# jontio/JAERO

Hardware: AMD Instinct MI355X
Metric: Msamples/s of real 48 kHz PCM through the 10.5 kbps OQPSK demodulator hot path (higher is better)
Workload: dtype f64; 1 GPU; 65536-channel-per-GPU synthetic 48 kHz 10.5 kbps OQPSK continuous (BASELINE configs[2] shape, scaled to 65536 channels per GPU = one wavefront of 64 channels per SIMD), 4096-sample writes, coarse 2^14 FFT every 4096 samples, AFC off, EbNo meters on, Eb/N0 10.0 dB, per-channel carrier (8000 +- 100 Hz), bits, noise, symbol phase; 42 untimed pre-roll steps (the last 14 resident and back to back with ; channels_per_gpu=65536, total_channels=65536, chunk=4096, ebno_meters=True, preroll_steps=42, timing_phases=32, hbm_bytes_per_resident_channel=2263808, resident_channels_max=136593, ranks=1, control_plane=none (single rank), sustain_steps=14

## Files before the change

### jaero_amd/csrc/k_coarse6.h

```cpp
#pragma once
#include "k_coarse2.h"

#ifndef C4_TABN
#define C4_TABN 3584
#endif
__device__ __forceinline__ void c6_bar() { asm volatile("s_waitcnt lgkmcnt(0)\n\ts_barrier" ::: "memory"); }
#define C6_FENCE __builtin_amdgcn_sched_barrier(0)
__device__ __forceinline__ double2 c6_sq(const double2 a)
{
#pragma clang fp contract(fast)
    return make_double2(a.x * a.x - a.y * a.y, 2.0 * (a.x * a.y));
}

#ifndef C6_TRACE
#define C6_TRACE(i)
#endif

template <int CTRL, int ROWMASK>
__device__ __forceinline__ void c6_argmax_step(double &bv, int &bi)
{
    const int lo = __builtin_amdgcn_update_dpp(__double2loint(bv), __double2loint(bv), CTRL, ROWMASK, 0xf, false);
    const int hi = __builtin_amdgcn_update_dpp(__double2hiint(bv), __double2hiint(bv), CTRL, ROWMASK, 0xf, false);
    const int oi = __builtin_amdgcn_update_dpp(bi, bi, CTRL, ROWMASK, 0xf, false);
    const double ov = __hiloint2double(hi, lo);
    const bool take = (oi >= 0) & ((bi < 0) | (ov > bv) | ((ov == bv) & (oi < bi)));
    bv = take ? ov : bv;
    bi = take ? oi : bi;
}
__device__ __forceinline__ void c6_wave_argmax(double &bv, int &bi)
{
    c6_argmax_step<0xB1, 0xf>(bv, bi);
    c6_argmax_step<0x4E, 0xf>(bv, bi);
    c6_argmax_step<0x141, 0xf>(bv, bi);
    c6_argmax_step<0x140, 0xf>(bv, bi);
    c6_argmax_step<0x142, 0xa>(bv, bi);
    c6_argmax_step<0x143, 0xc>(bv, bi);
    bv = __hiloint2double(__builtin_amdgcn_readlane(__double2hiint(bv), 63), __builtin_amdgcn_readlane(__double2loint(bv), 63));
    bi = __builtin_amdgcn_readlane(bi, 63);
}

#define C6_XCH 16448

__device__ __forceinline__ constexpr int c6_k(int s) { return s < 16 ? 2 * s : 2 * (s - 16) + 1; }

__device__ __forceinline__ void c6_fft32(CV<32> &x)
{
#pragma clang fp contract(fast)
#pragma unroll
    for (int j = 0; j < 16; j++)
    {
        const double ar = x.r[j], ai = x.i[j], br = x.r[j + 16], bi = x.i[j + 16];
        x.r[j] = ar + br; x.i[j] = ai + bi;
        double dr = ar - br, di = ai - bi;
        cmul_w64(dr, di, 2 * j);
        x.r[j + 16] = dr; x.i[j + 16] = di;
    }
    C6_FENCE;
#pragma unroll
    for (int h = 0; h < 2; h++)
    {
        CV<16> in, out;
#pragma unroll
        for (int j = 0; j < 16; j++) { in.r[j] = x.r[16 * h + j]; in.i[j] = x.i[16 * h + j]; }
        regfft<16>(in, out);
#pragma unroll
        for (int j = 0; j < 16; j++) { x.r[16 * h + j] = out.r[j]; x.i[16 * h + j] = out.i[j]; }
        C6_FENCE;
    }
}

__device__ __forceinline__ void c6_twiddle32(CV<32> &x, const double2 p1)
{
#pragma clang fp contract(fast)
    auto app = [&](int slot, const double2 w) __attribute__((always_inline)) {
        const double r = x.r[slot] * w.x - x.i[slot] * w.y, i = x.r[slot] * w.y + x.i[slot] * w.x;
        x.r[slot] = r; x.i[slot] = i;
    };
    const double2 p2 = c6_sq(p1);
    double2 e = p2;
    app(16, p1);
#pragma unroll
    for (int j = 1; j < 16; j++)
    {
        app(j, e);
        app(16 + j, cmul2(e, p1));
        if (j < 15) e = cmul2(e, p2);
    }
}

__device__ __forceinline__ void wg_fft14_e32(CV<32> &d, double *xch, const double2 *__restrict__ tw, int t)
{
#pragma clang fp contract(fast)
    const double2 st1 = tw[t], st2 = tw[32 * (t & 15)];
    const int k1u = t >> 4, n3 = t & 15, odd = k1u & 1;
    const int e1w0 = t, e1w1 = (t + 16) & 511;
    const int e1r = k1u * 512 + odd * 16 + n3;
    const int e1rw = e1r + 496 - 512 * odd;
    const int e2w = k1u + n3 * 513;
    const int e2r = t;

    c6_fft32(d);
    c6_twiddle32(d, st1);
    C6_FENCE;
    c6_bar();
#pragma unroll
    for (int s = 0; s < 32; s++) xch[c6_k(s) * 512 + ((c6_k(s) & 1) ? e1w1 : e1w0)] = d.r[s];
    c6_bar();
#pragma unroll
    for (int m = 0; m < 32; m++) d.r[m] = xch[(m < 31 ? e1r + 16 * m : e1rw)];
    c6_bar();
#pragma unroll
    for (int s = 0; s < 32; s++) xch[c6_k(s) * 512 + ((c6_k(s) & 1) ? e1w1 : e1w0)] = d.i[s];
    c6_bar();
#pragma unroll
    for (int m = 0; m < 32; m++) d.i[m] = xch[(m < 31 ? e1r + 16 * m : e1rw)];
    C6_FENCE;
    c6_fft32(d);
    c6_twiddle32(d, st2);
    C6_FENCE;
    c6_bar();
#pragma unroll
    for (int s = 0; s < 32; s++) xch[e2w + (c6_k(s) & 15) * 32 + (c6_k(s) >> 4) * 8208] = d.r[s];
    c6_bar();
#pragma unroll
    for (int m = 0; m < 32; m++) d.r[m] = xch[e2r + (m & 15) * 513 + (m >> 4) * 8208];
    c6_bar();
#pragma unroll
    for (int s = 0; s < 32; s++) xch[e2w + (c6_k(s) & 15) * 32 + (c6_k(s) >> 4) * 8208] = d.i[s];
    c6_bar();
#pragma unroll
    for (int m = 0; m < 32; m++) d.i[m] = xch[e2r + (m & 15) * 513 + (m >> 4) * 8208];
    C6_FENCE;
    {
        CV<16> in, o0, o1;
#pragma unroll
        for (int j = 0; j < 16; j++) { in.r[j] = d.r[j]; in.i[j] = d.i[j]; }
        regfft<16>(in, o0);
        C6_FENCE;
#pragma unroll
        for (int j = 0; j < 16; j++) { in.r[j] = d.r[16 + j]; in.i[j] = d.i[16 + j]; }
        regfft<16>(in, o1);
#pragma unroll
        for (int k3 = 0; k3 < 16; k3++) { d.r[2 * k3] = o0.r[k3]; d.i[2 * k3] = o0.i[k3]; d.r[2 * k3 + 1] = o1.r[k3]; d.i[2 * k3 + 1] = o1.i[k3]; }
    }
}


#define C6_XCH13 8208
__device__ __forceinline__ void wg_fft13_e32(CV<32> &d, double *xch, const double2 *__restrict__ tw, int t)
{
#pragma clang fp contract(fast)
    const double2 st1 = tw[t], st2 = tw[32 * (t & 15)];
    const int k1a = t >> 4, n3 = t & 15;
    const int e1r = k1a * 256 + n3;
    const int e2w = k1a + 513 * n3;
    c6_fft32(d);
    c6_twiddle32(d, st1);
    C6_FENCE;
    c6_bar();
#pragma unroll
    for (int s = 0; s < 32; s++) (xch + c6_k(s) * 256)[t] = d.r[s];
    c6_bar();
#pragma unroll
    for (int m = 0; m < 32; m++) d.r[m] = (xch + (m >> 4) * 4096 + (m & 15) * 16)[e1r];
    c6_bar();
#pragma unroll
    for (int s = 0; s < 32; s++) (xch + c6_k(s) * 256)[t] = d.i[s];
    c6_bar();
#pragma unroll
    for (int m = 0; m < 32; m++) d.i[m] = (xch + (m >> 4) * 4096 + (m & 15) * 16)[e1r];
    C6_FENCE;
#pragma unroll
    for (int g2 = 0; g2 < 2; g2++)
    {
        CV<16> in, out;
#pragma unroll
        for (int j = 0; j < 16; j++) { in.r[j] = d.r[16 * g2 + j]; in.i[j] = d.i[16 * g2 + j]; }
        regfft<16>(in, out);
        c4_twiddle16(out, st2);
#pragma unroll
        for (int j = 0; j < 16; j++) { d.r[16 * g2 + j] = out.r[j]; d.i[16 * g2 + j] = out.i[j]; }
        C6_FENCE;
    }
    c6_bar();
#pragma unroll
    for (int s = 0; s < 32; s++) (xch + (s >> 4) * 16 + (s & 15) * 32)[e2w] = d.r[s];
    c6_bar();
#pragma unroll
    for (int m = 0; m < 32; m++) d.r[m] = (xch + (m >> 4) * 256 + (m & 15) * 513)[t];
    c6_bar();
#pragma unroll
    for (int s = 0; s < 32; s++) (xch + (s >> 4) * 16 + (s & 15) * 32)[e2w] = d.i[s];
    c6_bar();
#pragma unroll
    for (int m = 0; m < 32; m++) d.i[m] = (xch + (m >> 4) * 256 + (m & 15) * 513)[t];
    C6_FENCE;
    {
        CV<16> in, o0, o1;
#pragma unroll
        for (int j = 0; j < 16; j++) { in.r[j] = d.r[j]; in.i[j] = d.i[j]; }
        regfft<16>(in, o0);
        C6_FENCE;
#pragma unroll
        for (int j = 0; j < 16; j++) { in.r[j] = d.r[16 + j]; in.i[j] = d.i[16 + j]; }
        regfft<16>(in, o1);
#pragma unroll
        for (int k3 = 0; k3 < 16; k3++) { d.r[2 * k3] = o0.r[k3]; d.i[2 * k3] = o0.i[k3]; d.r[2 * k3 + 1] = o1.r[k3]; d.i[2 * k3 + 1] = o1.i[k3]; }
    }
}

template <int LOG2N>
__device__ __forceinline__ void c6_fft(CV<32> &d, double *xch, const double2 *__restrict__ tw, int t)
{
    int tt = t;
    asm volatile("" : "+v"(tt));
    if constexpr (LOG2N == 14) wg_fft14_e32(d, xch, tw, tt);
    else wg_fft13_e32(d, xch, tw, tt);
}

__device__ __noinline__ void c6_build_window(double *wt, int startbin, int t, int nthreads)
{
    for (int i = t; i <= startbin + 1; i += nthreads)
    {
        const double c = cos(M_PI_2 * ((double)i) / ((double)startbin));
        wt[i] = (i == 0) ? 1.0 : ((i <= startbin) ? c * c : 0.0);
    }
}

template <bool W8400, int LOG2N = 14>
__device__ __forceinline__ void coarse6_body(const JGeom g, const JPtrs p, const int *__restrict__ chan_list, int nlist, const double2 *__restrict__ tw)
{
    constexpr int N = 1 << LOG2N;
    constexpr int E = 32;
    constexpr int NT = N / E;
    constexpr int XCH = LOG2N == 14 ? C6_XCH : C6_XCH13;
    extern __shared__ __attribute__((aligned(16))) double xch[];
    __shared__ double red_val[NT / 64];
    __shared__ int red_idx[NT / 64];
    const int t0 = threadIdx.x;
    const int nchp = g.nchp;
    int tab_startbin = -1;

    CV<E> d;
    int ch_next = ((int)blockIdx.x < nlist) ? (chan_list ? jd_sload(chan_list + blockIdx.x) : (int)blockIdx.x) : 0;
    int bp_next = jd_sload(p.I + (size_t)I_BB_PTR * nchp + ch_next);
    for (int li = blockIdx.x; li < nlist; li += gridDim.x)
    {
        int t = t0;
        asm volatile("" : "+v"(t));
        const int ch = ch_next, bb_ptr = bp_next;
        const double2 *__restrict__ ring = p.bbring + (size_t)ch * N;
        const int ln = li + (int)gridDim.x;
        const bool has_next = ln < nlist;
        if (has_next)
        {
            ch_next = chan_list ? jd_sload(chan_list + ln) : ln;
            bp_next = jd_sload(p.I + (size_t)I_BB_PTR * nchp + ch_next);
        }
        const double lockingbw = jd_sload(p.S + (size_t)S_LOCKINGBW * nchp + ch);
        double fs_l = g.Fs;
        asm volatile("" : "+s"(fs_l));
        int startbin, expectedpeakbin;
        {
            const double hzperbin = fs_l * (1.0 / ((double)N));
            startbin = __builtin_amdgcn_readfirstlane((int)fmax(round(lockingbw / hzperbin), 1.0));
            expectedpeakbin = __builtin_amdgcn_readfirstlane((int)round(g.fb / (2.0 * hzperbin)));
        }
        const int stopbin = N - startbin;
        double *__restrict__ y = p.y + (size_t)ch * N;

        if (li == (int)blockIdx.x)
        {
#pragma unroll
            for (int s = 0; s < E; s++)
            {
                const double2 v = ring[(bb_ptr + s * NT + t) & (N - 1)];
                d.r[s] = v.x; d.i[s] = v.y;
            }
        }
        C6_TRACE(0);
        c6_fft<LOG2N>(d, xch, tw, t);
        C6_TRACE(1);
        if constexpr (W8400)
        {
            const bool persistent = startbin < C4_TABN - 1;
            double *wt = persistent ? xch + XCH : xch;
            if (!persistent || startbin != tab_startbin)
            {
                c6_bar();
                c6_build_window(wt, startbin, t, NT);
                c6_bar();
                if (persistent) tab_startbin = startbin;
            }
#pragma unroll
            for (int s0 = 0; s0 < E; s0 += 8)
            {
#pragma unroll
                for (int s = s0; s < s0 + 8; s++)
                {
                    const int k = s * NT + t;
                    const int i = (k <= N / 2) ? k : N - k;
                    const double w = wt[i <= startbin ? i : startbin + 1];
                    const double re = d.r[s] * w, im = d.i[s] * w;
                    d.r[s] = im; d.i[s] = re;
                }
                C6_FENCE;
            }
            if (!persistent) c6_bar();
        }
        else
        {
#pragma unroll
            for (int s = 0; s < E; s++)
            {
                const int k = s * NT + t;
                const bool z = (k >= startbin) && (k <= stopbin);
                const double re = z ? 0.0 : d.r[s], im = z ? 0.0 : d.i[s];
                d.r[s] = im; d.i[s] = re;
            }
        }
        c6_fft<LOG2N>(d, xch, tw, t);
        C6_TRACE(2);
#pragma unroll
        for (int s = 0; s < E; s++)
        {
            const double re = d.i[s], im = d.r[s];
            d.r[s] = re * re - im * im;
            d.i[s] = re * im + im * re;
        }
        c6_fft<LOG2N>(d, xch, tw, t);
        C6_TRACE(3);
        c6_bar();
        CoarseSlotState cst;
        {
            double yv[E];
#pragma unroll
            for (int s = 0; s < E; s++) d.r[s] = d.r[s] * d.r[s] + d.i[s] * d.i[s];
            C6_FENCE;
#pragma unroll
            for (int s = 0; s < E; s++) yv[s] = __builtin_nontemporal_load((y + ((s * NT) ^ (N / 2))) + t);
            C6_FENCE;
            cst = coarse_slot_load_v(g, p, ch);
            int bpn = bp_next, chn = ch_next, tp = t;
            asm volatile("" : "+v"(bpn), "+v"(chn), "+v"(tp));
            typedef double c6_v2 __attribute__((ext_vector_type(2)));
            const c6_v2 *__restrict__ ringn = (const c6_v2 *)(p.bbring + (size_t)chn * N);
            const int toffp = bpn + tp;
#pragma unroll
            for (int s = 0; s < E; s++)
            {
                const int ib = (s * NT) ^ (N / 2);
                const double yn = yv[s] * 0.9 + 0.5 * jd_log10(fmax(d.r[s], 1.0));
                __builtin_nontemporal_store(yn, (y + ib) + t);
                (xch + ib)[t] = yn;
                {
                    const c6_v2 v = __builtin_nontemporal_load(ringn + ((toffp + s * NT) & (N - 1)));
                    d.r[s] = v.x; d.i[s] = v.y;
                }
                if ((s & 3) == 3) C6_FENCE;
            }
            C6_TRACE(4);
            c6_bar();
            C6_TRACE(5);
        }
        C6_TRACE(6);
        double fs_e = g.Fs;
        asm volatile("" : "+s"(fs_e));
        const double hzperbin = fs_e * (1.0 / ((double)N));
        const int i0 = __builtin_amdgcn_readfirstlane((int)round((-lockingbw / hzperbin) + ((double)(N / 2))));
        const int i1 = __builtin_amdgcn_readfirstlane((int)round((lockingbw / hzperbin) + ((double)(N / 2))));
        double best = 0;
        int besti = -1;
        const bool fold_inside = (i0 - expectedpeakbin - 1 >= 0) && (i1 + expectedpeakbin < N) && (i0 >= 0);
        if (fold_inside)
        {
            const int nblk = (i1 - i0 + 4 * NT - 1) / (4 * NT);
            for (int b = 0; b < nblk; b++)
            {
                double val[4];
#pragma unroll
                for (int u = 0; u < 4; u++)
                {
                    const int i = i0 + t + (4 * b + u) * NT;
                    const int ic = i < i1 ? i : i1 - 1;
                    const double *lo = xch + (ic - expectedpeakbin), *hi = xch + (ic + expectedpeakbin);
                    double v = 0;
                    v += (lo[1] + hi[-1]);
                    v += (lo[0] + hi[0]);
                    v += (lo[-1] + hi[1]);
                    val[u] = v;
                }
#pragma unroll
                for (int u = 0; u < 4; u++)
                {
                    const int i = i0 + t + (4 * b + u) * NT;
                    const bool take = (i < i1) & (val[u] > best);
                    best = take ? val[u] : best;
                    besti = take ? i : besti;
                }
            }
        }
        else
        {
            for (int i = i0 + t; i < i1; i += NT)
            {
                if ((i < 0) || (i >= N)) continue;
                double val = 0;
                for (int j = -1; j <= 1; j++)
                {
                    if (((i - expectedpeakbin - j) < 0) || ((i + expectedpeakbin + j) >= N)) continue;
                    val += (xch[i - expectedpeakbin - j] + xch[i + expectedpeakbin + j]);
                }
                if (val > best) { best = val; besti = i; }
            }
        }
        C6_TRACE(7);
        int bigchange;
        {
            double bv = best;
            int bi = besti;
            c6_wave_argmax(bv, bi);
            if ((t & 63) == 0) { red_val[t >> 6] = bv; red_idx[t >> 6] = bi; }
            C6_TRACE(8);
            c6_bar();
            bv = red_val[0]; bi = red_idx[0];
#pragma unroll
            for (int w = 1; w < NT / 64; w++)
            {
                const double ov = red_val[w];
                const int oi = red_idx[w];
                const bool take = (oi >= 0) & ((bi < 0) | (ov > bv) | ((ov == bv) & (oi < bi)));
                bv = take ? ov : bv;
                bi = take ? oi : bi;
            }
            bigchange = coarse_slot_apply(g, p, ch, cst, (bi >= 0) ? bi : (N / 2), N, hzperbin, lockingbw, t == 0);
            C6_TRACE(9);
        }
        if (bigchange)
        {
            __syncthreads();
            double2 *ringw = p.bbring + (size_t)ch * N;
            for (int i = t; i < N; i += NT) { y[i] = 20; ringw[i] = make_double2(0.0, 0.0); }
        }
        C6_TRACE(10);
    }
}

__global__ __launch_bounds__(C2_THREADS) void k_coarse6(const JGeom g, const JPtrs p, const int *__restrict__ chan_list,
                                                           int nlist, const double2 *__restrict__ tw)
{
    coarse6_body<false>(g, p, chan_list, nlist, tw);
}
__global__ __launch_bounds__(C2_THREADS) void k_coarse6_w8400(const JGeom g, const JPtrs p, const int *__restrict__ chan_list,
                                                                 int nlist, const double2 *__restrict__ tw)
{
    coarse6_body<true>(g, p, chan_list, nlist, tw);
}
__global__ __launch_bounds__(256, 2) void k_coarse6_13(const JGeom g, const JPtrs p, const int *__restrict__ chan_list,
                                                        int nlist, const double2 *__restrict__ tw)
{
    coarse6_body<false, 13>(g, p, chan_list, nlist, tw);
}
```

Baseline: 11700 Msamples/s.

## Prefetch coarse spectrum history into LDS during final FFT pass

The y spectrum history is now copied straight from global memory into LDS with global_load_lds_dwordx4, issued through a hook just before the last register-resident FFT pass, so the load overlaps FFT arithmetic instead of stalling after it. The baseband ring prefetch for the next channel is also split: a few loads go out early and the rest are interleaved with the y update loop. A counted vmcnt wait and an extra barrier coordinate this. The change relies on hand-written m0 and inline asm, and on a hard-coded outstanding-load count that could be fragile.

```diff
diff --git a/jaero_amd/csrc/k_coarse6.h b/jaero_amd/csrc/k_coarse6.h
--- a/jaero_amd/csrc/k_coarse6.h
+++ b/jaero_amd/csrc/k_coarse6.h
@@ -11,6 +11,17 @@
 #pragma clang fp contract(fast)
     return make_double2(a.x * a.x - a.y * a.y, 2.0 * (a.x * a.y));
 }
+
+#ifndef C6_Y_GLDS
+#define C6_Y_GLDS 1
+#endif
+#ifndef C6_Y_GLDS_CACHE
+#define C6_Y_GLDS_CACHE " nt"
+#endif
+#ifndef C6_RING_EARLY
+#define C6_RING_EARLY 4
+#endif
+struct C6NoHook { __device__ __forceinline__ void operator()() const {} };
 
 #ifndef C6_TRACE
 #define C6_TRACE(i)
@@ -88,7 +99,8 @@
     }
 }
 
-__device__ __forceinline__ void wg_fft14_e32(CV<32> &d, double *xch, const double2 *__restrict__ tw, int t)
+template <class HOOK>
+__device__ __forceinline__ void wg_fft14_e32(CV<32> &d, double *xch, const double2 *__restrict__ tw, int t, const HOOK &before_pass3)
 {
 #pragma clang fp contract(fast)
     const double2 st1 = tw[t], st2 = tw[32 * (t & 15)];
@@ -130,6 +142,7 @@
     c6_bar();
 #pragma unroll
     for (int m = 0; m < 32; m++) d.i[m] = xch[e2r + (m & 15) * 513 + (m >> 4) * 8208];
+    before_pass3();
     C6_FENCE;
     {
         CV<16> in, o0, o1;
@@ -147,7 +160,8 @@
 
 
 #define C6_XCH13 8208
-__device__ __forceinline__ void wg_fft13_e32(CV<32> &d, double *xch, const double2 *__restrict__ tw, int t)
+template <class HOOK>
+__device__ __forceinline__ void wg_fft13_e32(CV<32> &d, double *xch, const double2 *__restrict__ tw, int t, const HOOK &before_pass3)
 {
 #pragma clang fp contract(fast)
     const double2 st1 = tw[t], st2 = tw[32 * (t & 15)];
@@ -194,6 +208,7 @@
     c6_bar();
 #pragma unroll
     for (int m = 0; m < 32; m++) d.i[m] = (xch + (m >> 4) * 256 + (m & 15) * 513)[t];
+    before_pass3();
     C6_FENCE;
     {
         CV<16> in, o0, o1;
@@ -209,13 +224,34 @@
     }
 }
 
-template <int LOG2N>
-__device__ __forceinline__ void c6_fft(CV<32> &d, double *xch, const double2 *__restrict__ tw, int t)
+__device__ __forceinline__ void wg_fft14_e32(CV<32> &d, double *xch, const double2 *__restrict__ tw, int t) { wg_fft14_e32(d, xch, tw, t, C6NoHook()); }
+__device__ __forceinline__ void wg_fft13_e32(CV<32> &d, double *xch, const double2 *__restrict__ tw, int t) { wg_fft13_e32(d, xch, tw, t, C6NoHook()); }
+
+template <int LOG2N, class HOOK = C6NoHook>
+__device__ __forceinline__ void c6_fft(CV<32> &d, double *xch, const double2 *__restrict__ tw, int t, const HOOK &before_pass3 = HOOK())
 {
     int tt = t;
     asm volatile("" : "+v"(tt));
-    if constexpr (LOG2N == 14) wg_fft14_e32(d, xch, tw, tt);
-    else wg_fft13_e32(d, xch, tw, tt);
+    if constexpr (LOG2N == 14) wg_fft14_e32(d, xch, tw, tt, before_pass3);
+    else wg_fft13_e32(d, xch, tw, tt, before_pass3);
+}
+
+#define C6_Y_PIECES 16
+template <int N, int NT>
+__device__ __forceinline__ void c6_y_to_lds(const double *__restrict__ y, double *xch, int t)
+{
+    static_assert(N / 128 == C6_Y_PIECES * (NT / 64), "every wavefront issues C6_Y_PIECES pieces");
+    typedef __attribute__((address_space(3))) void *lds_ptr;
+    const int w = __builtin_amdgcn_readfirstlane(t >> 6);
+    const double *src = y + w * (C6_Y_PIECES * 128) + (t & 63) * 2;
+    const unsigned dst = __builtin_amdgcn_readfirstlane((unsigned)(size_t)(lds_ptr)(xch + w * (C6_Y_PIECES * 128)));
+#pragma unroll
+    for (int j = 0; j < C6_Y_PIECES; j++)
+    {
+        unsigned keep;
+        asm volatile("s_mov_b32 %0, m0\n\ts_mov_b32 m0, %2\n\ts_nop 0\n\tglobal_load_lds_dwordx4 %1, off" C6_Y_GLDS_CACHE "\n\ts_mov_b32 m0, %0"
+                     : "=&s"(keep) : "v"(src + j * 128), "s"(dst + j * 1024) : "memory");
+    }
 }
 
 __device__ __noinline__ void c6_build_window(double *wt, int startbin, int t, int nthreads)
@@ -328,9 +364,52 @@
             d.r[s] = re * re - im * im;
             d.i[s] = re * im + im * re;
         }
+#if C6_Y_GLDS
+        c6_fft<LOG2N>(d, xch, tw, t, [&]() __attribute__((always_inline)) { c6_bar(); c6_y_to_lds<N, NT>(y, xch, t); });
+#else
         c6_fft<LOG2N>(d, xch, tw, t);
+#endif
         C6_TRACE(3);
+#if C6_Y_GLDS
+        CoarseSlotState cst;
+        {
+            constexpr int E0 = C6_RING_EARLY;
+            static_assert(E0 >= 0 && E0 <= E && 13 + E0 <= 63, "the counted wait below");
+#pragma unroll
+            for (int s = 0; s < E; s++) d.r[s] = d.r[s] * d.r[s] + d.i[s] * d.i[s];
+            C6_FENCE;
+            cst = coarse_slot_load_v(g, p, ch);
+            int bpn = bp_next, chn = ch_next, tp = t;
+            asm volatile("" : "+v"(bpn), "+v"(chn), "+v"(tp));
+            typedef double c6_v2 __attribute__((ext_vector_type(2)));
+            const c6_v2 *__restrict__ ringn = (const c6_v2 *)(p.bbring + (size_t)chn * N);
+            const int toffp = bpn + tp;
+            c6_v2 nx[E];
+#pragma unroll
+            for (int k = 0; k < E0; k++) nx[k] = __builtin_nontemporal_load(ringn + ((toffp + k * NT) & (N - 1)));
+            C6_FENCE;
+            asm volatile("s_waitcnt vmcnt(%0)" ::"n"(13 + E0) : "memory");
+            c6_bar();
+            C6_TRACE(11);
+#pragma unroll
+            for (int s = 0; s < E; s++)
+            {
+                const int ib = (s * NT) ^ (N / 2);
+                const double yn = (xch + ib)[t] * 0.9 + 0.5 * jd_log10(fmax(d.r[s], 1.0));
+                __builtin_nontemporal_store(yn, (y + ib) + t);
+                (xch + ib)[t] = yn;
+#pragma unroll
+                for (int k = E0 + (s * (E - E0)) / E; k < E0 + ((s + 1) * (E - E0)) / E; k++)
+                    nx[k] = __builtin_nontemporal_load(ringn + ((toffp + k * NT) & (N - 1)));
+                if ((s & 3) == 3) C6_FENCE;
+            }
+#pragma unroll
+            for (int s = 0; s < E; s++) { d.r[s] = nx[s].x; d.i[s] = nx[s].y; }
+            asm volatile("" : "+v"(cst.emptying), "+v"(cst.flags), "+v"(cst.countdown), "+v"(cst.countdown2), "+v"(cst.nest), "+v"(cst.log_cnt));
+            asm volatile("" : "+v"(cst.mse), "+v"(cst.thr), "+v"(cst.m2_freq), "+v"(cst.m2_step), "+v"(cst.mc_freq), "+v"(cst.mc_step), "+v"(cst.ebno));
+#else
         c6_bar();
+        C6_TRACE(11);
         CoarseSlotState cst;
         {
             double yv[E];
@@ -359,6 +438,7 @@
                 }
                 if ((s & 3) == 3) C6_FENCE;
             }
+#endif
             C6_TRACE(4);
             c6_bar();
             C6_TRACE(5);
```

Result: no change. 11810 Msamples/s, median of 6 (+1.0%).
